# paganpasta/eqxvision

Hardware: AMD Instinct MI355X
Metric: images/sec (higher is better)
Workload: dtype bf16; 1 GPU; resnet50 bf16 forward, batch=256/GPU, 3x224x224, 1000 classes; global_batch=256, parallelism=dp1, graph=True, lanes=2, collective_forced_1rank=False

## Files before the change

eqxvision_amd/build.py:

```python
from __future__ import annotations

import glob
import os
import subprocess
import sys
from concurrent.futures import ThreadPoolExecutor

HERE = os.path.dirname(os.path.abspath(__file__))
CSRC = os.path.join(HERE, "csrc")
LIB = os.path.join(CSRC, "libeqxvision_amd.so")
HIPCC = os.environ.get("HIPCC", "/opt/rocm/bin/hipcc")
FLAGS = ["--offload-arch=gfx950", "-O3", "-std=c++17", "-fPIC", "-Wno-unused-value"]
PROF = bool(os.environ.get("EQV_PROF"))
if PROF:
    FLAGS.append("-DMV_I8_PROF")
    LIB = os.path.join(CSRC, "libeqxvision_amd_prof.so")


def _newer(src, dst):
    return (not os.path.exists(dst)) or os.path.getmtime(src) > os.path.getmtime(dst)


def build(force: bool = False, verbose: bool = True) -> str:
    srcs = sorted(glob.glob(os.path.join(CSRC, "*.hip")))
    hdrs = glob.glob(os.path.join(CSRC, "*.h")) + glob.glob(os.path.join(HERE, "..", "include", "*.h"))
    objdir = os.path.join(CSRC, "build_prof" if PROF else "build")
    os.makedirs(objdir, exist_ok=True)
    newest_hdr = max(os.path.getmtime(h) for h in hdrs)
    jobs = []
    for s in srcs:
        o = os.path.join(objdir, os.path.basename(s)[:-4] + ".o")
        if force or _newer(s, o) or newest_hdr > os.path.getmtime(o):
            jobs.append((s, o))

    def cc(job):
        s, o = job
        cmd = [HIPCC] + FLAGS + ["-c", s, "-o", o]
        r = subprocess.run(cmd, capture_output=True, text=True)
        if r.returncode != 0:
            raise RuntimeError(f"hipcc failed on {s}:\n{r.stderr[-4000:]}")
        return s

    if jobs:
        if verbose:
            print(f"[eqxvision_amd.build] compiling {len(jobs)} file(s) for gfx950", file=sys.stderr)
        with ThreadPoolExecutor(max_workers=min(8, len(jobs))) as ex:
            list(ex.map(cc, jobs))
    objs = [os.path.join(objdir, os.path.basename(s)[:-4] + ".o") for s in srcs]
    if jobs or not os.path.exists(LIB):
        r = subprocess.run([HIPCC, "--offload-arch=gfx950", "-shared", "-fPIC"] + objs + ["-ldl", "-o", LIB],
                           capture_output=True, text=True)
        if r.returncode != 0:
            raise RuntimeError(f"link failed:\n{r.stderr[-4000:]}")
    return LIB


if __name__ == "__main__":
    print(build(force="--force" in sys.argv))
```

eqxvision_amd/csrc/igemm8.hip:

```cpp
#include <type_traits>

#include "igemm_pipe.h"

namespace mv {

namespace {

constexpr unsigned OOB = 0x80000000u;

__device__ unsigned g_dev_status = 0;
constexpr int LDS_W = 0, LDS_XT = 65536, LDS_XB = 98304;
constexpr int LDS_TOTAL = 131072;
constexpr int LDS_LNP = LDS_TOTAL, LN_MAXP = 3, LDS_LNS = LDS_LNP + LN_MAXP * 2048, LDS_TOTAL_LN = LDS_LNS + 2048;
constexpr int LDS_LN_SLOTS = 8 * 32 * (64 * 4 + 16), LDS_LN_DUMMY = LDS_LN_SLOTS + 256 * 32;
static_assert(LDS_LN_DUMMY + 8 * 512 <= LDS_TOTAL, "producer statistics slots");

template <int LOFF>
__device__ __forceinline__ void dma16(unsigned ldsw, unsigned voff, const u32x4& rsrc, unsigned soff) {
    asm volatile("s_add_u32 m0, %0, %4\n\tbuffer_load_dwordx4 %1, %2, %3 offen lds"
                 :
                 : "s"(ldsw), "v"(voff), "s"(rsrc), "s"(soff), "n"(LOFF)
                 : "memory", "scc");
}

template <int LOFF>
__device__ __forceinline__ void dma4(unsigned ldsw, unsigned voff, const u32x4& rsrc, unsigned soff) {
    asm volatile("s_add_u32 m0, %0, %4\n\tbuffer_load_dword %1, %2, %3 offen lds"
                 :
                 : "s"(ldsw), "v"(voff), "s"(rsrc), "s"(soff), "n"(LOFF)
                 : "memory", "scc");
}

__device__ __forceinline__ u32x4 make_rsrc(const void* base) {
    const unsigned long long b = (unsigned long long)base;
    u32x4 r;
    r[0] = __builtin_amdgcn_readfirstlane((unsigned)b);
    r[1] = __builtin_amdgcn_readfirstlane((unsigned)(b >> 32) & 0xffffu);
    r[2] = OOB;
    r[3] = 0x00020000u;
    return r;
}

template <int N> __device__ __forceinline__ void wait_vm_lgkm0() {
    asm volatile("s_waitcnt vmcnt(%0) lgkmcnt(0)" ::"n"(N) : "memory");
}

}

struct TapState {
    int r, s, c0;
    unsigned xoff;
    unsigned woff;
    unsigned bit;
};

__device__ __forceinline__ TapState tap_first() {
    TapState s;
    s.r = 0; s.s = 0; s.c0 = 0; s.xoff = 0; s.woff = 0; s.bit = 1u;
    return s;
}

template <bool DUAL> __device__ __forceinline__ void tap_next(const Igemm2P& p, TapState& s, int tile, int nk1) {
    s.woff += 128u;
    if (DUAL && tile >= nk1) {
        s.xoff = 128u * (unsigned)(tile - nk1);
        return;
    }
    s.c0 += 64;
    if (s.c0 == p.C) {
        s.c0 = 0;
        if (++s.s == p.S) { s.s = 0; ++s.r; }
        s.bit <<= 1;
    }
    s.xoff = 2u * (unsigned)(((s.r * p.dh) * p.W + s.s * p.dw) * p.C + s.c0);
}

template <bool DUAL> __device__ __forceinline__ TapState tap_at(const Igemm2P& p, int tile, int nk1) {
// ... 131 lines not shown
    for (int j = 0; j < 4; ++j) {
        const int n = n0 + 64 * j + 8 * wave + srow;
        wvo[j] = n < p.K ? (unsigned)n * wrow_bytes + 16u * (unsigned)gch : OOB;
    }
    const unsigned lds0 = (unsigned)(uintptr_t)(__attribute__((address_space(3))) char*)smem;
    const unsigned ldsw = __builtin_amdgcn_readfirstlane(lds0 + wave * (8 * ROWB));

    auto tap_adv = [&](TapState& s, int tile) {
        if constexpr (DENSE) { s.woff += 128u; s.xoff += 128u; }
        else tap_next<DUAL>(p, s, tile, nk1);
    };
    auto x_piece = [&](int q, const TapState& s, int tile, auto loff) {
        constexpr int LOFF = decltype(loff)::value;
        if (DUAL && tile >= nk1) {
            if constexpr (DUAL) dma16<LOFF>(ldsw, xvo2[q], rx2, s.xoff);
        } else if constexpr (DENSE) {
            dma16<LOFF>(ldsw, xvo[q], rx, s.xoff);
        } else {
            const unsigned vo = (xmask[q] & s.bit) ? xvo[q] : OOB;
            dma16<LOFF>(ldsw, vo, rx, s.xoff);
        }
    };
#define MV_I8_W(BUF, st)                                                           \
    do {                                                                           \
        dma16<LDS_W + (BUF) * 32768 + 0 * 8192>(ldsw, wvo[0], rw, (st).woff);      \
        dma16<LDS_W + (BUF) * 32768 + 1 * 8192>(ldsw, wvo[1], rw, (st).woff);      \
        dma16<LDS_W + (BUF) * 32768 + 2 * 8192>(ldsw, wvo[2], rw, (st).woff);      \
        dma16<LDS_W + (BUF) * 32768 + 3 * 8192>(ldsw, wvo[3], rw, (st).woff);      \
    } while (0)
#define MV_I8_X(BUF, q, st, tile)                                                                                     \
    x_piece(q, st, tile,                                                                                               \
            std::integral_constant<int, ((q) < 2 ? LDS_XT : LDS_XB) + (BUF) * 16384 + ((q) & 1) * 8192>{})

    const int fr = lane & 31, fh = lane >> 5, swz = (fr >> 1) & 7;
    unsigned waddr[4], xaddr[4];
#pragma unroll
    for (int kk = 0; kk < 4; ++kk) {
        const unsigned ko = (unsigned)(((2 * kk + fh) ^ swz) << 4);
        waddr[kk] = lds0 + LDS_W + (64 * wc + fr) * ROWB + ko;
        xaddr[kk] = lds0 + LDS_XT + (64 * grp + fr) * ROWB + ko;
    }

#ifdef MV_I8_PROF
    const OutT* res = (p.dbg & 8) ? nullptr : (const OutT*)p.residual;
    const bool do_store = !(p.dbg & 4);
#else
    const OutT* res = (const OutT*)p.residual;
    constexpr bool do_store = true;
#endif
    ScaleShift8 ss;
    if constexpr (LIN) ss.load_shift(p.shift, n0 + 64 * wc + (lane & 7) * 8, p.K);
    else ss.load(p.scale, p.shift, n0 + 64 * wc + (lane & 7) * 8, p.K);

    f32x16 acc[2][4];
#pragma unroll
    for (int a = 0; a < 2; ++a)
#pragma unroll
        for (int b = 0; b < 4; ++b)
#pragma unroll
            for (int e = 0; e < 16; ++e) acc[a][b][e] = 0.f;

    TapState sa = tap_first();
    TapState sb = tap_first();
    if constexpr (LNF == 2) {
        const u32x4 rs = make_rsrc(p.stats_in);
        const unsigned ldsw4 = __builtin_amdgcn_readfirstlane(lds0 + wave * 256);
        const unsigned svo = m0 + (tid >> 1) < p.M ? 4u * (unsigned)(2 * m0 + tid) : OOB;
        const unsigned pstep = 8u * (unsigned)p.M;
        const int P = (p.C + 255) >> 8;
#define MV_I8_LNP(j) if ((j) < P) dma4<LDS_LNP + (j) * 2048>(ldsw4, svo, rs, (unsigned)(j) * pstep)
        MV_I8_LNP(0); MV_I8_LNP(1); MV_I8_LNP(2);
#undef MV_I8_LNP
    }
    MV_I8_W(0, sa);
    MV_I8_X(0, 0, sa, 0);
    MV_I8_X(0, 1, sb, 0);
    MV_I8_X(0, 2, sb, 0);
    MV_I8_X(0, 3, sb, 0);
    auto ln_finalize = [&]() {
        __builtin_amdgcn_s_barrier();
        if (tid < 256) {
            const int P = (p.C + 255) >> 8;
            const unsigned a0 = lds0 + LDS_LNP + 8u * (unsigned)tid;
            u32x2 pc[LN_MAXP];
#define MV_I8_RD(j) asm volatile("ds_read_b64 %0, %1 offset:%2" : "=v"(pc[j]) : "v"(a0), "n"((j) * 2048) : "memory")
            MV_I8_RD(0); MV_I8_RD(1); MV_I8_RD(2);
#undef MV_I8_RD
            asm volatile("s_waitcnt lgkmcnt(0)" ::: "memory");
#pragma unroll
            for (int j = 0; j < LN_MAXP; ++j) asm volatile("" : "+v"(pc[j]));
            float tot = 0.f;
#pragma unroll
            for (int j = 0; j < LN_MAXP; ++j) tot += j < P ? __uint_as_float(pc[j][0]) : 0.f;
            const float inv_n = 1.0f / (float)p.C, mean = tot * inv_n;
            float m2 = 0.f;
#pragma unroll
            for (int j = 0; j < LN_MAXP; ++j) {
                const float nj = (float)min(256, p.C - 256 * j);
                const float d = __uint_as_float(pc[j][0]) / nj - mean;
                m2 += j < P ? __uint_as_float(pc[j][1]) + nj * d * d : 0.f;
            }
            const float rstd = 1.0f / sqrtf(m2 * inv_n + p.ln_eps);
            *(float2*)(smem + LDS_LNS + 8 * tid) = make_float2(-mean * rstd, rstd);
        }
    };
    if (nk > 1) {
        tap_adv(sa, 1);
        MV_I8_W(1, sa);
        MV_I8_X(1, 0, sa, 1);
        if constexpr (LNF == 2) { wait_vm<13>(); ln_finalize(); }
        wait_vm<7>();
    } else {
        if constexpr (LNF == 2) { wait_vm<8>(); ln_finalize(); }
        wait_vm<2>();
    }
    __builtin_amdgcn_s_barrier();
    if (grp == 1) __builtin_amdgcn_s_barrier();
#ifdef MV_I8_PROF
    if (p.prof) pt1 = wall_clock64();
#endif
    MV_I8_STAMP();

    u32x4 wf[2][4], xf[2][4];
    auto mfma_half = [&](int half) {
        __builtin_amdgcn_sched_barrier(0);
        __builtin_amdgcn_s_setprio(1);
#pragma unroll
        for (int kk = 0; kk < 4; ++kk)
#pragma unroll
            for (int a = 0; a < 2; ++a)
#pragma unroll
                for (int b = 0; b < 2; ++b)
                    acc[a][2 * half + b] = __builtin_amdgcn_mfma_f32_32x32x16_bf16(
                        __builtin_bit_cast(bf16x8, wf[a][kk]), __builtin_bit_cast(bf16x8, xf[b][kk]), acc[a][2 * half + b], 0, 0, 0);
        __builtin_amdgcn_s_setprio(0);
        __builtin_amdgcn_sched_barrier(0);
    };
    auto pin_frags = [&]() {
#pragma unroll
        for (int kk = 0; kk < 4; ++kk)
            asm volatile("" : "+v"(wf[0][kk]), "+v"(wf[1][kk]), "+v"(xf[0][kk]), "+v"(xf[1][kk]));
    };

    auto ktile = [&](int it, auto bufc) {
        constexpr int BUF = decltype(bufc)::value;
#ifdef MV_I8_PROF
        const bool do_reads = !(p.dbg & 2), do_dma = !(p.dbg & 1);
#else
        constexpr bool do_reads = true, do_dma = true;
#endif
        if (do_reads) {
#pragma unroll
            for (int kk = 0; kk < 4; ++kk) {
                lds_read16<BUF * 32768>(wf[0][kk], waddr[kk]);
                lds_read16<BUF * 32768 + 32 * ROWB>(wf[1][kk], waddr[kk]);
            }
#pragma unroll
            for (int kk = 0; kk < 4; ++kk) {
                lds_read16<BUF * 16384>(xf[0][kk], xaddr[kk]);
                lds_read16<BUF * 16384 + 32 * ROWB>(xf[1][kk], xaddr[kk]);
            }
        }
        if (!do_dma) {
            wait_vm_lgkm0<0>();
        } else if (it + 1 < nk) {
            tap_adv(sb, it + 1);
            MV_I8_X(BUF ^ 1, 1, sb, it + 1);
            MV_I8_X(BUF ^ 1, 2, sb, it + 1);
            MV_I8_X(BUF ^ 1, 3, sb, it + 1);
            wait_vm_lgkm0<8>();
        } else {
            wait_vm_lgkm0<0>();
        }
        pin_frags();
        __builtin_amdgcn_s_barrier();
        MV_I8_STAMP();
        mfma_half(0);
        __builtin_amdgcn_s_barrier();
        MV_I8_STAMP();
        if (do_reads) {
#pragma unroll
            for (int kk = 0; kk < 4; ++kk) {
                lds_read16<(LDS_XB - LDS_XT) + BUF * 16384>(xf[0][kk], xaddr[kk]);
                lds_read16<(LDS_XB - LDS_XT) + BUF * 16384 + 32 * ROWB>(xf[1][kk], xaddr[kk]);
            }
        }
        if (!do_dma) {
            wait_vm_lgkm0<0>();
        } else if (it + 2 < nk) {
            tap_adv(sa, it + 2);
            MV_I8_W(BUF, sa);
            MV_I8_X(BUF, 0, sa, it + 2);
            wait_vm_lgkm0<7>();
        } else if (it + 1 < nk) {
            wait_vm_lgkm0<2>();
        } else {
            wait_vm_lgkm0<0>();
        }
        pin_frags();
        __builtin_amdgcn_s_barrier();
        MV_I8_STAMP();
        mfma_half(1);
        __builtin_amdgcn_s_barrier();
        MV_I8_STAMP();
    };
    for (int it = 0; it < nk; it += 2) {
        ktile(it, std::integral_constant<int, 0>{});
        if (it + 1 < nk) ktile(it + 1, std::integral_constant<int, 1>{});
    }
    if (grp == 0) __builtin_amdgcn_s_barrier();
#ifdef MV_I8_PROF
    if (p.prof) pt2 = wall_clock64();
#endif

    if constexpr (LNF == 0 || LNF == 2)
        epilogue_rows<OutT, LIN, 4, EPITCH, LNF>(p, smem + wave * (32 * EPITCH), acc, ss, res, do_store, m0 + 128 * grp, n0 + 64 * wc, lane,
                                                 smem + LDS_LNS + 1024 * grp);
    else
    {
        epilogue_rows_ln<LNF != 1, LNF != 4, 4, EPITCH>(p, smem + wave * (32 * EPITCH), acc, ss, do_store, m0 + 128 * grp, n0 + 64 * wc, lane,
                                                        smem + LDS_LN_SLOTS + 128 * 32 * grp, wc, smem + LDS_LN_DUMMY + 512 * wave);
        if constexpr (LNF != 4) {
            __syncthreads();
            if (tid < 256 && do_store) merge_row_stats(p, smem + LDS_LN_SLOTS, tid, m0, tile_n, min(4, (p.K - n0) >> 6));
        }
    }
#ifdef MV_I8_PROF
    if (p.prof) {
        if (tid == 0) {
            long long* o = p.prof + 4ll * blockIdx.x;
            o[0] = pt0; o[1] = pt1; o[2] = pt2; o[3] = wall_clock64();
        }
        if (blockIdx.x == 0 && lane == 0) {
            long long* o = p.prof + 4ll * gridDim.x + wave * 128;
            for (int i = 0; i < 128; ++i) o[i] = i < nstamp ? (long long)stamps[i] : -1;
        }
    }
#endif
#undef MV_I8_STAMP
#undef MV_I8_W
#undef MV_I8_X
}

template <typename OutT, int ARR, bool DUAL, bool DENSE = false>
__global__ __launch_bounds__(512) void igemm8s_kernel(const Igemm2P p) {
    static_assert(!(DUAL && DENSE), "DENSE is single-source");
    constexpr int BM = ARR == 0 ? 128 : 256, BN = ARR == 0 ? 256 : 128;
    constexpr int ROWB = 128;
    constexpr int XI = BM / 64, WI = BN / 64;
    constexpr int XBYTES = BM * ROWB;
    constexpr int SLOT = (BM + BN) * ROWB;
    constexpr int EPITCH = 64 * 4 + 16;
    static_assert(XI + WI == 6 && 3 * SLOT <= 160 * 1024 && 8 * 32 * EPITCH <= 3 * SLOT, "ring layout");
// ... 52 lines not shown
        const bool second = DUAL && tile >= nk1;
        if (second) {
            if constexpr (DUAL) {
                dma16<BASE + 0 * 8192>(ldsw, xvo2[0], rx2, st.xoff);
                dma16<BASE + 1 * 8192>(ldsw, xvo2[1], rx2, st.xoff);
                if constexpr (XI == 4) {
                    dma16<BASE + 2 * 8192>(ldsw, xvo2[2], rx2, st.xoff);
                    dma16<BASE + 3 * 8192>(ldsw, xvo2[3], rx2, st.xoff);
                }
            }
        } else if constexpr (DENSE) {
            dma16<BASE + 0 * 8192>(ldsw, xvo[0], rx, st.xoff);
            dma16<BASE + 1 * 8192>(ldsw, xvo[1], rx, st.xoff);
            if constexpr (XI == 4) {
                dma16<BASE + 2 * 8192>(ldsw, xvo[2], rx, st.xoff);
                dma16<BASE + 3 * 8192>(ldsw, xvo[3], rx, st.xoff);
            }
        } else {
            dma16<BASE + 0 * 8192>(ldsw, (xmask[0] & st.bit) ? xvo[0] : OOB, rx, st.xoff);
            dma16<BASE + 1 * 8192>(ldsw, (xmask[1] & st.bit) ? xvo[1] : OOB, rx, st.xoff);
            if constexpr (XI == 4) {
                dma16<BASE + 2 * 8192>(ldsw, (xmask[2] & st.bit) ? xvo[2] : OOB, rx, st.xoff);
                dma16<BASE + 3 * 8192>(ldsw, (xmask[3] & st.bit) ? xvo[3] : OOB, rx, st.xoff);
            }
        }
        dma16<BASE + XBYTES + 0 * 8192>(ldsw, wvo[0], rw, st.woff);
        dma16<BASE + XBYTES + 1 * 8192>(ldsw, wvo[1], rw, st.woff);
        if constexpr (WI == 4) {
            dma16<BASE + XBYTES + 2 * 8192>(ldsw, wvo[2], rw, st.woff);
            dma16<BASE + XBYTES + 3 * 8192>(ldsw, wvo[3], rw, st.woff);
        }
    };

    const int fr = lane & 31, fh = lane >> 5, swz = (fr >> 1) & 7;
    unsigned waddr[4], xaddr[4], waddr2[4], xaddr2[4];
#pragma unroll
    for (int kk = 0; kk < 4; ++kk) {
        const unsigned ko = (unsigned)(((2 * kk + fh) ^ swz) << 4);
        xaddr[kk] = lds0 + (xrow0 + fr) * ROWB + ko;
        waddr[kk] = lds0 + XBYTES + (wrow0 + fr) * ROWB + ko;
        xaddr2[kk] = xaddr[kk] + 2 * SLOT;
        waddr2[kk] = waddr[kk] + 2 * SLOT;
    }

    const OutT* res = (const OutT*)p.residual;
    ScaleShift8 ss;
    ss.load(p.scale, p.shift, n0 + wrow0 + (lane & 7) * 8, p.K);

    f32x16 acc[2][2];
#pragma unroll
    for (int a = 0; a < 2; ++a)
#pragma unroll
        for (int b = 0; b < 2; ++b)
#pragma unroll
            for (int e = 0; e < 16; ++e) acc[a][b][e] = 0.f;

    TapState st = tap_first();
    if (k0) {
        if constexpr (DENSE) { st.woff = st.xoff = 128u * (unsigned)k0; }
        else st = tap_at<DUAL>(p, k0, nk1);
    }
    stage(st, k0, std::integral_constant<int, 0>{});
    if (nk > 1) {
        tap_adv(st, k0 + 1);
        stage(st, k0 + 1, std::integral_constant<int, 1>{});
        wait_vm<6>();
    } else {
        wait_vm<0>();
    }
    __builtin_amdgcn_s_barrier();
    if (grp == 1) __builtin_amdgcn_s_barrier();

    u32x4 wf[2][4], xf[2][4];
    auto ktile = [&](int it, auto slotc) {
        constexpr int SL = decltype(slotc)::value;
        constexpr int OFF = SL == 2 ? 0 : SL * SLOT;
#pragma unroll
        for (int kk = 0; kk < 4; ++kk) {
            lds_read16<OFF>(wf[0][kk], SL == 2 ? waddr2[kk] : waddr[kk]);
            lds_read16<OFF + 32 * ROWB>(wf[1][kk], SL == 2 ? waddr2[kk] : waddr[kk]);
            lds_read16<OFF>(xf[0][kk], SL == 2 ? xaddr2[kk] : xaddr[kk]);
            lds_read16<OFF + 32 * ROWB>(xf[1][kk], SL == 2 ? xaddr2[kk] : xaddr[kk]);
        }
        if (it + 2 < nk) {
            tap_adv(st, k0 + it + 2);
            stage(st, k0 + it + 2, std::integral_constant<int, (SL + 2) % 3>{});
            wait_vm_lgkm0<6>();
        } else {
            wait_vm_lgkm0<0>();
        }
#pragma unroll
        for (int kk = 0; kk < 4; ++kk)
            asm volatile("" : "+v"(wf[0][kk]), "+v"(wf[1][kk]), "+v"(xf[0][kk]), "+v"(xf[1][kk]));
        __builtin_amdgcn_s_barrier();
        __builtin_amdgcn_sched_barrier(0);
        __builtin_amdgcn_s_setprio(1);
#pragma unroll
        for (int kk = 0; kk < 4; ++kk)
#pragma unroll
            for (int a = 0; a < 2; ++a)
#pragma unroll
                for (int b = 0; b < 2; ++b)
                    acc[a][b] = __builtin_amdgcn_mfma_f32_32x32x16_bf16(__builtin_bit_cast(bf16x8, wf[a][kk]),
                                                                        __builtin_bit_cast(bf16x8, xf[b][kk]), acc[a][b], 0, 0, 0);
        __builtin_amdgcn_s_setprio(0);
        __builtin_amdgcn_sched_barrier(0);
        __builtin_amdgcn_s_barrier();
    };
    for (int it = 0; it < nk; it += 3) {
        ktile(it, std::integral_constant<int, 0>{});
        if (it + 1 < nk) ktile(it + 1, std::integral_constant<int, 1>{});
        if (it + 2 < nk) ktile(it + 2, std::integral_constant<int, 2>{});
    }
    if (grp == 0) __builtin_amdgcn_s_barrier();

    if (splitk) {
        unsigned* sync = p.sync + 2 * t;
        float4* part = (float4*)p.ws + (size_t)t * (BM * BN / 4) + tid;
        const unsigned xcc = __builtin_amdgcn_s_getreg(20 | (3 << 11)) & 15u;
        if (tid == 0) *(volatile unsigned*)smem = __hip_atomic_fetch_add(sync, 1u, __ATOMIC_RELAXED, __HIP_MEMORY_SCOPE_AGENT);
        __syncthreads();
        const unsigned arrived = *(volatile unsigned*)smem;
        __syncthreads();
        if (arrived == 0) {
#pragma unroll
            for (int a = 0; a < 2; ++a)
#pragma unroll
                for (int b = 0; b < 2; ++b)
#pragma unroll
                    for (int g = 0; g < 4; ++g)
                        part[((a * 2 + b) * 4 + g) * 512] = make_float4(acc[a][b][4 * g + 0], acc[a][b][4 * g + 1],
                                                                        acc[a][b][4 * g + 2], acc[a][b][4 * g + 3]);
            __syncthreads();
            if (tid == 0) __hip_atomic_store(sync + 1, 1u + xcc, __ATOMIC_RELEASE, __HIP_MEMORY_SCOPE_AGENT);
            return;
        }
        if (tid == 0) {
            int spins = 0;
            unsigned f;
            while ((f = __hip_atomic_load(sync + 1, __ATOMIC_RELAXED, __HIP_MEMORY_SCOPE_AGENT)) == 0u && ++spins < (1 << 20))
                __builtin_amdgcn_s_sleep(2);
            if (f == 0u)
                __hip_atomic_fetch_or(&g_dev_status, 1u, __ATOMIC_RELAXED, __HIP_MEMORY_SCOPE_AGENT);
            if (f != 1u + xcc) __builtin_amdgcn_fence(__ATOMIC_ACQUIRE, "agent");
            __hip_atomic_store(sync, 0u, __ATOMIC_RELAXED, __HIP_MEMORY_SCOPE_AGENT);
            __hip_atomic_store(sync + 1, 0u, __ATOMIC_RELAXED, __HIP_MEMORY_SCOPE_AGENT);
        }
        __syncthreads();
#pragma unroll
        for (int a = 0; a < 2; ++a)
#pragma unroll
            for (int b = 0; b < 2; ++b)
#pragma unroll
                for (int g = 0; g < 4; ++g) {
                    const float4 o = part[((a * 2 + b) * 4 + g) * 512];
                    acc[a][b][4 * g + 0] += o.x; acc[a][b][4 * g + 1] += o.y; acc[a][b][4 * g + 2] += o.z; acc[a][b][4 * g + 3] += o.w;
                }
    }

    epilogue_rows<OutT, false, 2, EPITCH>(p, smem + wave * (32 * EPITCH), acc, ss, res, true, m0 + xrow0, n0 + wrow0, lane);
}

int device_status(int clear, unsigned* out) {
    unsigned v = 0;
    MV_HIP(hipMemcpyFromSymbol(&v, HIP_SYMBOL(g_dev_status), sizeof(v), 0, hipMemcpyDeviceToHost));
    if (clear && v) {
        const unsigned z = 0;
        MV_HIP(hipMemcpyToSymbol(HIP_SYMBOL(g_dev_status), &z, sizeof(z), 0, hipMemcpyHostToDevice));
    }
    *out = v;
    return MV_OK;
}

unsigned* device_status_word() {
    void* p = nullptr;
    if (hipGetSymbolAddress(&p, HIP_SYMBOL(g_dev_status)) != hipSuccess) {
        (void)hipGetLastError();
        return nullptr;
    }
    return (unsigned*)p;
}

size_t splitk_scratch_bytes(long long M, long long N, long long kred) {
    if (N <= 0 || M <= 0) return 0;
    const long long ta = ((M + 127) / 128) * ((N + 255) / 256), tb = ((M + 255) / 256) * ((N + 127) / 128);
    if (!splitk_rule(ta < tb ? ta : tb, kred / 64, get_flag)) return 0;
    return SPLITK_SYNC_BYTES + (size_t)(ta > tb ? ta : tb) * 128 * 256 * 4;
}

static int igemm8_go(Igemm2P& p, bool dual, bool out_f32, int tile, hipStream_t st) {
    const int bm = tile == 1 ? 128 : 256, bn = tile == 2 ? 128 : 256;
    p.tiles_m = (p.M + bm - 1) / bm;
    p.tiles_n = (p.K + bn - 1) / bn;
// ... 157 lines not shown
```

eqxvision_amd/csrc/igemm_pipe.h:

```cpp
#pragma once
#include "mfma_common.h"

namespace mv {

struct Igemm2P {
    const bf16_t* x;
    const bf16_t* w;
    const float* scale;
    const float* shift;
    const void* residual;
    void* y;
    const bf16_t* zero;
    int N, H, W, C, K, R, S, Ho, Wo, sh, sw, ph, pw, dh, dw;
    int M, tiles_m, tiles_n, act;
    int dbg;
    long long* prof;
    const bf16_t* x2;
    int C2, H2, W2, s2;
    int gm;
    int skew;
    int tok;
    unsigned* sync;
    float* ws;
    void* y2;
    const void* residual2;
    float* stats_out;
    const float* stats_in;
    float ln_eps;
};

typedef unsigned int u32x4 __attribute__((ext_vector_type(4)));
typedef unsigned int u32x2 __attribute__((ext_vector_type(2)));

template <int IMM> __device__ __forceinline__ void lds_read16(u32x4& dst, unsigned addr) {
    asm volatile("ds_read_b128 %0, %1 offset:%2" : "=v"(dst) : "v"(addr), "n"(IMM) : "memory");
}
template <int N> __device__ __forceinline__ void wait_vm() { asm volatile("s_waitcnt vmcnt(%0)" ::"n"(N) : "memory"); }

template <typename OutT> struct R8;
template <> struct R8<bf16_t> {
    uint4 u;
    __device__ __forceinline__ void load(const bf16_t* p) { u = *(const uint4*)p; }
    __device__ __forceinline__ void add_to(float* v) const {
        const uint32_t w[4] = {u.x, u.y, u.z, u.w};
#pragma unroll
        for (int e = 0; e < 4; ++e) {
            v[2 * e] += __uint_as_float(w[e] << 16);
            v[2 * e + 1] += __uint_as_float(w[e] & 0xffff0000u);
        }
    }
};
template <> struct R8<float> {
    float4 a, b;
    __device__ __forceinline__ void load(const float* p) { a = *(const float4*)p; b = *(const float4*)(p + 4); }
    __device__ __forceinline__ void add_to(float* v) const {
        v[0] += a.x; v[1] += a.y; v[2] += a.z; v[3] += a.w; v[4] += b.x; v[5] += b.y; v[6] += b.z; v[7] += b.w;
    }
};


template <typename OutT> struct Buf8;
template <> struct Buf8<bf16_t> {
    u32x4 u;
    __device__ __forceinline__ void load(brsrc_t r, unsigned vo, unsigned so) { u = __builtin_amdgcn_raw_buffer_load_b128(r, vo, so, 0); }
    __device__ __forceinline__ void add_to(float* v) const {
// ... 8 lines not shown
        o[0] = pack_bf2(v[0], v[1]); o[1] = pack_bf2(v[2], v[3]); o[2] = pack_bf2(v[4], v[5]); o[3] = pack_bf2(v[6], v[7]);
        __builtin_amdgcn_raw_buffer_store_b128(o, r, vo, 0, 0);
    }
};
template <> struct Buf8<float> {
    u32x4 a, b;
    __device__ __forceinline__ void load(brsrc_t r, unsigned vo, unsigned so) {
        a = __builtin_amdgcn_raw_buffer_load_b128(r, vo, so, 0);
        b = __builtin_amdgcn_raw_buffer_load_b128(r, vo + 16u, so, 0);
    }
    __device__ __forceinline__ void add_to(float* v) const {
#pragma unroll
        for (int e = 0; e < 4; ++e) { v[e] += __uint_as_float(a[e]); v[4 + e] += __uint_as_float(b[e]); }
    }
    static __device__ __forceinline__ void store(brsrc_t r, unsigned vo, const float* v) {
        u32x4 lo, hi;
#pragma unroll
        for (int e = 0; e < 4; ++e) { lo[e] = __float_as_uint(v[e]); hi[e] = __float_as_uint(v[4 + e]); }
        __builtin_amdgcn_raw_buffer_store_b128(lo, r, vo, 0, 0);
        __builtin_amdgcn_raw_buffer_store_b128(hi, r, vo + 16u, 0, 0);
    }
};

__device__ __forceinline__ float dpp_xor1(float v) { return __builtin_bit_cast(float, __builtin_amdgcn_update_dpp(0, __builtin_bit_cast(int, v), 0xB1, 0xf, 0xf, true)); }
__device__ __forceinline__ float dpp_xor2(float v) { return __builtin_bit_cast(float, __builtin_amdgcn_update_dpp(0, __builtin_bit_cast(int, v), 0x4E, 0xf, 0xf, true)); }
__device__ __forceinline__ float dpp_half_mirror(float v) { return __builtin_bit_cast(float, __builtin_amdgcn_update_dpp(0, __builtin_bit_cast(int, v), 0x141, 0xf, 0xf, true)); }
__device__ __forceinline__ float sum8_lanes(float v) {
    v += dpp_xor1(v);
    v += dpp_xor2(v);
    v += dpp_half_mirror(v);
    return v;
}

template <typename OutT, bool LIN, int NBT, int EPITCH, int LNF = 0>
__device__ __forceinline__ void epilogue_rows(const Igemm2P& p, char* ep, f32x16 (&acc)[2][NBT], const ScaleShift8& ss,
                                              const OutT* res, bool do_store, int mrow0, int ncol0, int lane,
                                              const char* lnst = nullptr) {
    static_assert(LNF == 0 || (LNF == 2 && sizeof(OutT) == 2 && !LIN), "LayerNorm fold, consumer form");
    constexpr unsigned SZ = sizeof(OutT);
    const int fr = lane & 31, fh = lane >> 5, r0 = lane >> 3, c8 = lane & 7;
    const int rl = ncol0 + c8 * 8 < p.K ? p.M - mrow0 : 0;
    const long long wave_elem = (long long)mrow0 * p.K + ncol0;
    const bool has_res = res != nullptr;
    const brsrc_t rr = make_brsrc(has_res ? res + wave_elem : (const OutT*)p.y, has_res);
    const unsigned vrow = (unsigned)(r0 * p.K + c8 * 8) * SZ;
    const unsigned kstep = 8u * (unsigned)p.K * SZ;
    const bool hm = p.tok > 0;
    int bi0 = 0, ti0 = 0;
    if (hm) { bi0 = mrow0 / p.tok; ti0 = mrow0 - bi0 * p.tok; }
    const long long y_elem = hm ? ((long long)bi0 * (p.K >> 6) + (ncol0 >> 6)) * p.tok * 64 : wave_elem;
    const brsrc_t ry = make_brsrc((OutT*)p.y + y_elem, do_store);
    const float inv_tok = hm ? 1.0f / (float)p.tok : 0.f;
    const unsigned img_step = (unsigned)(p.K >> 6) * (unsigned)p.tok * 64u;
    auto row_vo = [&](int row) -> unsigned { return row + r0 < rl ? vrow : BUF_OOB; };
    auto y_vo = [&](int row, int step) -> unsigned {
        unsigned rel = vrow + (unsigned)step * kstep;
        if (hm) {
            const int v = ti0 + row + r0;
            int q = (int)((float)v * inv_tok), t = v - q * p.tok;
            q += t >= p.tok ? 1 : (t < 0 ? -1 : 0);
            t -= t >= p.tok ? p.tok : (t < 0 ? -p.tok : 0);
            rel = ((unsigned)q * img_step + (unsigned)t * 64u + (unsigned)c8 * 8u) * SZ;
        }
        return row + r0 < rl ? rel : BUF_OOB;
    };
    Buf8<OutT> late[2][4];
    auto fetch_res = [&](int b, Buf8<OutT>(&dst)[4]) {
#pragma unroll
        for (int pass = 0; pass < 4; ++pass) dst[pass].load(rr, row_vo(b * 32 + pass * 8), (unsigned)(b * 4 + pass) * kstep);
    };
    fetch_res(0, late[0]);
#pragma unroll
    for (int b = 0; b < NBT; ++b) {
        if (b + 1 < NBT) fetch_res(b + 1, late[(b + 1) & 1]);
#pragma unroll
        for (int a = 0; a < 2; ++a)
#pragma unroll
            for (int g = 0; g < 4; ++g) {
                const int nl = a * 32 + 8 * g + 4 * fh;
                *(float4*)(ep + fr * EPITCH + nl * 4) = make_float4(acc[a][b][4 * g + 0], acc[a][b][4 * g + 1],
                                                                     acc[a][b][4 * g + 2], acc[a][b][4 * g + 3]);
            }
        wave_lds_fence();
#pragma unroll
        for (int pass = 0; pass < 4; ++pass) {
            const int row = pass * 8 + r0;
            const float4 lo = *(const float4*)(ep + row * EPITCH + c8 * 32);
            const float4 hi = *(const float4*)(ep + row * EPITCH + c8 * 32 + 16);
            float v[8] = {lo.x, lo.y, lo.z, lo.w, hi.x, hi.y, hi.z, hi.w};
            if constexpr (LNF == 2) {
                const float2 st = *(const float2*)(lnst + (b * 32 + row) * 8);
#pragma unroll
                for (int e = 0; e < 8; ++e) v[e] = fmaf(st.y, v[e], fmaf(st.x, ss.sc[e], ss.sh[e]));
            } else if constexpr (LIN) ss.apply_shift(v);
            else ss.apply(v);
            if (has_res) late[b & 1][pass].add_to(v);
            const unsigned voy = y_vo(b * 32 + pass * 8, b * 4 + pass);
            if (p.act == MV_ACT_RELU) {
#pragma unroll
                for (int e = 0; e < 8; ++e) v[e] = fmaxf(v[e], 0.f);
            }
            if constexpr (sizeof(OutT) == 2) {
                u32x4 o;
                if (p.act == MV_ACT_GELU_TANH) {
                    o[0] = gelu_tanh_pack2(v[0], v[1]); o[1] = gelu_tanh_pack2(v[2], v[3]);
                    o[2] = gelu_tanh_pack2(v[4], v[5]); o[3] = gelu_tanh_pack2(v[6], v[7]);
                } else {
                    o[0] = pack_bf2(v[0], v[1]); o[1] = pack_bf2(v[2], v[3]); o[2] = pack_bf2(v[4], v[5]); o[3] = pack_bf2(v[6], v[7]);
                }
                __builtin_amdgcn_raw_buffer_store_b128(o, ry, voy, 0, 0);
            } else {
                if (p.act == MV_ACT_GELU_TANH) {
#pragma unroll
                    for (int e = 0; e < 8; ++e) v[e] = gelu_tanh_f(v[e]);
                }
                Buf8<OutT>::store(ry, voy, v);
            }
        }
        wave_lds_fence();
    }
}


template <bool RES_SPLIT, bool OUT_SPLIT, int NBT, int EPITCH>
__device__ __forceinline__ void epilogue_rows_ln(const Igemm2P& p, char* ep, f32x16 (&acc)[2][NBT], const ScaleShift8& ss, bool do_store,
                                                 int mrow0, int ncol0, int lane, char* slots, int wc, char* dummy) {
    static_assert(RES_SPLIT || OUT_SPLIT, "fp32 in, fp32 out is the plain epilogue");
    const int fr = lane & 31, fh = lane >> 5, r0 = lane >> 3, c8 = lane & 7;
    const int rl = ncol0 + c8 * 8 < p.K ? p.M - mrow0 : 0;
    const long long wave_elem = (long long)mrow0 * p.K + ncol0;
    const unsigned vrow2 = (unsigned)(r0 * p.K + c8 * 8) * 2u, kstep2 = 16u * (unsigned)p.K;
    const brsrc_t rra = make_brsrc(RES_SPLIT ? (const void*)((const bf16_t*)p.residual + wave_elem) : (const void*)((const float*)p.residual + wave_elem));
    const brsrc_t rrb = make_brsrc(RES_SPLIT ? (const void*)((const bf16_t*)p.residual2 + wave_elem) : (const void*)p.y, RES_SPLIT);
    const brsrc_t rya = make_brsrc(OUT_SPLIT ? (void*)((bf16_t*)p.y + wave_elem) : (void*)((float*)p.y + wave_elem), do_store);
    const brsrc_t ryb = make_brsrc(OUT_SPLIT ? (void*)((bf16_t*)p.y2 + wave_elem) : p.y, OUT_SPLIT && do_store);
    auto row_ok = [&](int row) -> bool { return row + r0 < rl; };
    u32x4 la[2][4], lb[2][4];
    auto fetch_res = [&](int b, u32x4 (&da)[4], u32x4 (&db)[4]) {
#pragma unroll
        for (int pass = 0; pass < 4; ++pass) {
            const bool ok = row_ok(b * 32 + pass * 8);
            const unsigned step = (unsigned)(b * 4 + pass);
            if constexpr (RES_SPLIT) {
                da[pass] = __builtin_amdgcn_raw_buffer_load_b128(rra, ok ? vrow2 : BUF_OOB, step * kstep2, 0);
                db[pass] = __builtin_amdgcn_raw_buffer_load_b128(rrb, ok ? vrow2 : BUF_OOB, step * kstep2, 0);
            } else {
                da[pass] = __builtin_amdgcn_raw_buffer_load_b128(rra, ok ? 2u * vrow2 : BUF_OOB, step * 2u * kstep2, 0);
                db[pass] = __builtin_amdgcn_raw_buffer_load_b128(rra, ok ? 2u * vrow2 + 16u : BUF_OOB, step * 2u * kstep2, 0);
            }
        }
    };
    fetch_res(0, la[0], lb[0]);
#pragma unroll
    for (int b = 0; b < NBT; ++b) {
        if (b + 1 < NBT) fetch_res(b + 1, la[(b + 1) & 1], lb[(b + 1) & 1]);
#pragma unroll
        for (int a = 0; a < 2; ++a)
#pragma unroll
            for (int g = 0; g < 4; ++g) {
                const int nl = a * 32 + 8 * g + 4 * fh;
                *(float4*)(ep + fr * EPITCH + nl * 4) = make_float4(acc[a][b][4 * g + 0], acc[a][b][4 * g + 1],
                                                                     acc[a][b][4 * g + 2], acc[a][b][4 * g + 3]);
            }
        wave_lds_fence();
#pragma unroll
        for (int pass = 0; pass < 4; ++pass) {
            const int row = pass * 8 + r0;
            const float4 lo = *(const float4*)(ep + row * EPITCH + c8 * 32);
            const float4 hi = *(const float4*)(ep + row * EPITCH + c8 * 32 + 16);
            float v[8] = {lo.x, lo.y, lo.z, lo.w, hi.x, hi.y, hi.z, hi.w};
            ss.apply_shift(v);
            const u32x4 ra = la[b & 1][pass], rb = lb[b & 1][pass];
#pragma unroll
            for (int e = 0; e < 4; ++e) {
                if constexpr (RES_SPLIT) {
                    v[2 * e] += __uint_as_float(ra[e] << 16) + __uint_as_float(rb[e] << 16);
                    v[2 * e + 1] += __uint_as_float(ra[e] & 0xffff0000u) + __uint_as_float(rb[e] & 0xffff0000u);
                } else {
                    v[e] += __uint_as_float(ra[e]);
                    v[4 + e] += __uint_as_float(rb[e]);
                }
            }
            const bool ok = row_ok(b * 32 + pass * 8);
            const unsigned step = (unsigned)(b * 4 + pass);
            if constexpr (OUT_SPLIT) {
                const float s = sum8_lanes(((v[0] + v[1]) + (v[2] + v[3])) + ((v[4] + v[5]) + (v[6] + v[7])));
                const float mu = s * (1.0f / 64.0f);
                float q = 0.f;
#pragma unroll
                for (int e = 0; e < 8; ++e) { const float d = v[e] - mu; q = fmaf(d, d, q); }
                q = sum8_lanes(q);
                *(float2*)(c8 == 0 ? slots + ((b * 32 + row) * 4 + wc) * 8 : dummy + lane * 8) = make_float2(s, q);
                u32x4 oh, ol;
#pragma unroll
                for (int e = 0; e < 4; ++e) {
                    oh[e] = pack_bf2(v[2 * e], v[2 * e + 1]);
// ... 35 lines not shown
```

Before: 90620 images/s.

## Switch implicit-GEMM inner loop from 32x32x16 to 16x16x32 bf16 MFMA

```diff
diff --git a/eqxvision_amd/build.py b/eqxvision_amd/build.py
--- a/eqxvision_amd/build.py
+++ b/eqxvision_amd/build.py
@@ -15,6 +15,11 @@
 if PROF:
     FLAGS.append("-DMV_I8_PROF")
     LIB = os.path.join(CSRC, "libeqxvision_amd_prof.so")
+OBJDIR = "build_prof" if PROF else "build"
+if os.environ.get("EQV_I8_M16") == "0":
+    FLAGS.append("-DMV_I8_M16=0")
+    LIB = LIB[:-3] + "_m32.so"
+    OBJDIR += "_m32"
 
 
 def _newer(src, dst):
@@ -24,7 +29,7 @@
 def build(force: bool = False, verbose: bool = True) -> str:
     srcs = sorted(glob.glob(os.path.join(CSRC, "*.hip")))
     hdrs = glob.glob(os.path.join(CSRC, "*.h")) + glob.glob(os.path.join(HERE, "..", "include", "*.h"))
-    objdir = os.path.join(CSRC, "build_prof" if PROF else "build")
+    objdir = os.path.join(CSRC, OBJDIR)
     os.makedirs(objdir, exist_ok=True)
     newest_hdr = max(os.path.getmtime(h) for h in hdrs)
     jobs = []
diff --git a/eqxvision_amd/csrc/igemm8.hip b/eqxvision_amd/csrc/igemm8.hip
--- a/eqxvision_amd/csrc/igemm8.hip
+++ b/eqxvision_amd/csrc/igemm8.hip
@@ -1,6 +1,10 @@
 #include <type_traits>
 
 #include "igemm_pipe.h"
+
+#ifndef MV_I8_M16
+#define MV_I8_M16 1
+#endif
 
 namespace mv {
 
@@ -43,6 +47,17 @@
 
 template <int N> __device__ __forceinline__ void wait_vm_lgkm0() {
     asm volatile("s_waitcnt vmcnt(%0) lgkmcnt(0)" ::"n"(N) : "memory");
+}
+
+constexpr bool M16 = MV_I8_M16 != 0;
+constexpr int FROWS = M16 ? 16 : 32, FT = 64 / FROWS, KS = M16 ? 2 : 4, FCH = 8 / KS, LAY = M16 ? 1 : 0;
+using acc_t = std::conditional_t<M16, f32x4, f32x16>;
+__device__ __forceinline__ acc_t mfma_step(const u32x4& w, const u32x4& x, const acc_t& c) {
+#if MV_I8_M16
+    return __builtin_amdgcn_mfma_f32_16x16x32_bf16(__builtin_bit_cast(bf16x8, w), __builtin_bit_cast(bf16x8, x), c, 0, 0, 0);
+#else
+    return __builtin_amdgcn_mfma_f32_32x32x16_bf16(__builtin_bit_cast(bf16x8, w), __builtin_bit_cast(bf16x8, x), c, 0, 0, 0);
+#endif
 }
 
 }
@@ -240,11 +255,11 @@
     x_piece(q, st, tile,                                                                                               \
             std::integral_constant<int, ((q) < 2 ? LDS_XT : LDS_XB) + (BUF) * 16384 + ((q) & 1) * 8192>{})
 
-    const int fr = lane & 31, fh = lane >> 5, swz = (fr >> 1) & 7;
-    unsigned waddr[4], xaddr[4];
-#pragma unroll
-    for (int kk = 0; kk < 4; ++kk) {
-        const unsigned ko = (unsigned)(((2 * kk + fh) ^ swz) << 4);
+    const int fr = lane & (FROWS - 1), fh = lane / FROWS, swz = (fr >> 1) & 7;
+    unsigned waddr[KS], xaddr[KS];
+#pragma unroll
+    for (int kk = 0; kk < KS; ++kk) {
+        const unsigned ko = (unsigned)(((FCH * kk + fh) ^ swz) << 4);
         waddr[kk] = lds0 + LDS_W + (64 * wc + fr) * ROWB + ko;
         xaddr[kk] = lds0 + LDS_XT + (64 * grp + fr) * ROWB + ko;
     }
@@ -260,13 +275,13 @@
     if constexpr (LIN) ss.load_shift(p.shift, n0 + 64 * wc + (lane & 7) * 8, p.K);
     else ss.load(p.scale, p.shift, n0 + 64 * wc + (lane & 7) * 8, p.K);
 
-    f32x16 acc[2][4];
-#pragma unroll
-    for (int a = 0; a < 2; ++a)
-#pragma unroll
-        for (int b = 0; b < 4; ++b)
-#pragma unroll
-            for (int e = 0; e < 16; ++e) acc[a][b][e] = 0.f;
+    acc_t acc[FT][2 * FT];
+#pragma unroll
+    for (int a = 0; a < FT; ++a)
+#pragma unroll
+        for (int b = 0; b < 2 * FT; ++b)
+#pragma unroll
+            for (int e = 0; e < (int)(sizeof(acc_t) / 4); ++e) acc[a][b][e] = 0.f;
 
     TapState sa = tap_first();
     TapState sb = tap_first();
@@ -329,25 +344,38 @@
 #endif
     MV_I8_STAMP();
 
-    u32x4 wf[2][4], xf[2][4];
+    u32x4 wf[FT][KS], xf[FT][KS];
     auto mfma_half = [&](int half) {
         __builtin_amdgcn_sched_barrier(0);
         __builtin_amdgcn_s_setprio(1);
 #pragma unroll
-        for (int kk = 0; kk < 4; ++kk)
-#pragma unroll
-            for (int a = 0; a < 2; ++a)
-#pragma unroll
-                for (int b = 0; b < 2; ++b)
-                    acc[a][2 * half + b] = __builtin_amdgcn_mfma_f32_32x32x16_bf16(
-                        __builtin_bit_cast(bf16x8, wf[a][kk]), __builtin_bit_cast(bf16x8, xf[b][kk]), acc[a][2 * half + b], 0, 0, 0);
+        for (int kk = 0; kk < KS; ++kk)
+#pragma unroll
+            for (int a = 0; a < FT; ++a)
+#pragma unroll
+                for (int b = 0; b < FT; ++b)
+                    acc[a][FT * half + b] = mfma_step(wf[a][kk], xf[b][kk], acc[a][FT * half + b]);
         __builtin_amdgcn_s_setprio(0);
         __builtin_amdgcn_sched_barrier(0);
     };
     auto pin_frags = [&]() {
 #pragma unroll
-        for (int kk = 0; kk < 4; ++kk)
-            asm volatile("" : "+v"(wf[0][kk]), "+v"(wf[1][kk]), "+v"(xf[0][kk]), "+v"(xf[1][kk]));
+        for (int kk = 0; kk < KS; ++kk)
+#pragma unroll
+            for (int t = 0; t < FT; t += 2)
+                asm volatile("" : "+v"(wf[t][kk]), "+v"(wf[t + 1][kk]), "+v"(xf[t][kk]), "+v"(xf[t + 1][kk]));
+    };
+    auto read_frags = [&](u32x4 (&f)[FT][KS], const unsigned (&addr)[KS], auto basec) {
+        constexpr int BASE = decltype(basec)::value;
+#pragma unroll
+        for (int kk = 0; kk < KS; ++kk) {
+            lds_read16<BASE>(f[0][kk], addr[kk]);
+            lds_read16<BASE + FROWS * ROWB>(f[1][kk], addr[kk]);
+            if constexpr (FT == 4) {
+                lds_read16<BASE + 2 * FROWS * ROWB>(f[2][kk], addr[kk]);
+                lds_read16<BASE + 3 * FROWS * ROWB>(f[3][kk], addr[kk]);
+            }
+        }
     };
 
     auto ktile = [&](int it, auto bufc) {
@@ -358,16 +386,8 @@
         constexpr bool do_reads = true, do_dma = true;
 #endif
         if (do_reads) {
-#pragma unroll
-            for (int kk = 0; kk < 4; ++kk) {
-                lds_read16<BUF * 32768>(wf[0][kk], waddr[kk]);
-                lds_read16<BUF * 32768 + 32 * ROWB>(wf[1][kk], waddr[kk]);
-            }
-#pragma unroll
-            for (int kk = 0; kk < 4; ++kk) {
-                lds_read16<BUF * 16384>(xf[0][kk], xaddr[kk]);
-                lds_read16<BUF * 16384 + 32 * ROWB>(xf[1][kk], xaddr[kk]);
-            }
+            read_frags(wf, waddr, std::integral_constant<int, BUF * 32768>{});
+            read_frags(xf, xaddr, std::integral_constant<int, BUF * 16384>{});
         }
         if (!do_dma) {
             wait_vm_lgkm0<0>();
@@ -386,13 +406,7 @@
         mfma_half(0);
         __builtin_amdgcn_s_barrier();
         MV_I8_STAMP();
-        if (do_reads) {
-#pragma unroll
-            for (int kk = 0; kk < 4; ++kk) {
-                lds_read16<(LDS_XB - LDS_XT) + BUF * 16384>(xf[0][kk], xaddr[kk]);
-                lds_read16<(LDS_XB - LDS_XT) + BUF * 16384 + 32 * ROWB>(xf[1][kk], xaddr[kk]);
-            }
-        }
+        if (do_reads) read_frags(xf, xaddr, std::integral_constant<int, (LDS_XB - LDS_XT) + BUF * 16384>{});
         if (!do_dma) {
             wait_vm_lgkm0<0>();
         } else if (it + 2 < nk) {
@@ -422,11 +436,11 @@
 #endif
 
     if constexpr (LNF == 0 || LNF == 2)
-        epilogue_rows<OutT, LIN, 4, EPITCH, LNF>(p, smem + wave * (32 * EPITCH), acc, ss, res, do_store, m0 + 128 * grp, n0 + 64 * wc, lane,
+        epilogue_rows<OutT, LIN, 4, EPITCH, LNF, LAY>(p, smem + wave * (32 * EPITCH), acc, ss, res, do_store, m0 + 128 * grp, n0 + 64 * wc, lane,
                                                  smem + LDS_LNS + 1024 * grp);
     else
     {
-        epilogue_rows_ln<LNF != 1, LNF != 4, 4, EPITCH>(p, smem + wave * (32 * EPITCH), acc, ss, do_store, m0 + 128 * grp, n0 + 64 * wc, lane,
+        epilogue_rows_ln<LNF != 1, LNF != 4, 4, EPITCH, LAY>(p, smem + wave * (32 * EPITCH), acc, ss, do_store, m0 + 128 * grp, n0 + 64 * wc, lane,
                                                         smem + LDS_LN_SLOTS + 128 * 32 * grp, wc, smem + LDS_LN_DUMMY + 512 * wave);
         if constexpr (LNF != 4) {
             __syncthreads();
@@ -545,11 +559,11 @@
         }
     };
 
-    const int fr = lane & 31, fh = lane >> 5, swz = (fr >> 1) & 7;
-    unsigned waddr[4], xaddr[4], waddr2[4], xaddr2[4];
-#pragma unroll
-    for (int kk = 0; kk < 4; ++kk) {
-        const unsigned ko = (unsigned)(((2 * kk + fh) ^ swz) << 4);
+    const int fr = lane & (FROWS - 1), fh = lane / FROWS, swz = (fr >> 1) & 7;
+    unsigned waddr[KS], xaddr[KS], waddr2[KS], xaddr2[KS];
+#pragma unroll
+    for (int kk = 0; kk < KS; ++kk) {
+        const unsigned ko = (unsigned)(((FCH * kk + fh) ^ swz) << 4);
         xaddr[kk] = lds0 + (xrow0 + fr) * ROWB + ko;
         waddr[kk] = lds0 + XBYTES + (wrow0 + fr) * ROWB + ko;
         xaddr2[kk] = xaddr[kk] + 2 * SLOT;
@@ -560,13 +574,13 @@
     ScaleShift8 ss;
     ss.load(p.scale, p.shift, n0 + wrow0 + (lane & 7) * 8, p.K);
 
-    f32x16 acc[2][2];
-#pragma unroll
-    for (int a = 0; a < 2; ++a)
-#pragma unroll
-        for (int b = 0; b < 2; ++b)
-#pragma unroll
-            for (int e = 0; e < 16; ++e) acc[a][b][e] = 0.f;
+    acc_t acc[FT][FT];
+#pragma unroll
+    for (int a = 0; a < FT; ++a)
+#pragma unroll
+        for (int b = 0; b < FT; ++b)
+#pragma unroll
+            for (int e = 0; e < (int)(sizeof(acc_t) / 4); ++e) acc[a][b][e] = 0.f;
 
     TapState st = tap_first();
     if (k0) {
@@ -584,16 +598,25 @@
     __builtin_amdgcn_s_barrier();
     if (grp == 1) __builtin_amdgcn_s_barrier();
 
-    u32x4 wf[2][4], xf[2][4];
+    u32x4 wf[FT][KS], xf[FT][KS];
     auto ktile = [&](int it, auto slotc) {
         constexpr int SL = decltype(slotc)::value;
         constexpr int OFF = SL == 2 ? 0 : SL * SLOT;
 #pragma unroll
-        for (int kk = 0; kk < 4; ++kk) {
-            lds_read16<OFF>(wf[0][kk], SL == 2 ? waddr2[kk] : waddr[kk]);
-            lds_read16<OFF + 32 * ROWB>(wf[1][kk], SL == 2 ? waddr2[kk] : waddr[kk]);
-            lds_read16<OFF>(xf[0][kk], SL == 2 ? xaddr2[kk] : xaddr[kk]);
-            lds_read16<OFF + 32 * ROWB>(xf[1][kk], SL == 2 ? xaddr2[kk] : xaddr[kk]);
+        for (int kk = 0; kk < KS; ++kk) {
+            const unsigned wa = SL == 2 ? waddr2[kk] : waddr[kk], xa = SL == 2 ? xaddr2[kk] : xaddr[kk];
+            lds_read16<OFF>(wf[0][kk], wa);
+            lds_read16<OFF + FROWS * ROWB>(wf[1][kk], wa);
+            if constexpr (FT == 4) {
+                lds_read16<OFF + 2 * FROWS * ROWB>(wf[2][kk], wa);
+                lds_read16<OFF + 3 * FROWS * ROWB>(wf[3][kk], wa);
+            }
+            lds_read16<OFF>(xf[0][kk], xa);
+            lds_read16<OFF + FROWS * ROWB>(xf[1][kk], xa);
+            if constexpr (FT == 4) {
+                lds_read16<OFF + 2 * FROWS * ROWB>(xf[2][kk], xa);
+                lds_read16<OFF + 3 * FROWS * ROWB>(xf[3][kk], xa);
+            }
         }
         if (it + 2 < nk) {
             tap_adv(st, k0 + it + 2);
@@ -603,19 +626,19 @@
             wait_vm_lgkm0<0>();
         }
 #pragma unroll
-        for (int kk = 0; kk < 4; ++kk)
-            asm volatile("" : "+v"(wf[0][kk]), "+v"(wf[1][kk]), "+v"(xf[0][kk]), "+v"(xf[1][kk]));
+        for (int kk = 0; kk < KS; ++kk)
+#pragma unroll
+            for (int t = 0; t < FT; t += 2)
+                asm volatile("" : "+v"(wf[t][kk]), "+v"(wf[t + 1][kk]), "+v"(xf[t][kk]), "+v"(xf[t + 1][kk]));
         __builtin_amdgcn_s_barrier();
         __builtin_amdgcn_sched_barrier(0);
         __builtin_amdgcn_s_setprio(1);
 #pragma unroll
-        for (int kk = 0; kk < 4; ++kk)
-#pragma unroll
-            for (int a = 0; a < 2; ++a)
-#pragma unroll
-                for (int b = 0; b < 2; ++b)
-                    acc[a][b] = __builtin_amdgcn_mfma_f32_32x32x16_bf16(__builtin_bit_cast(bf16x8, wf[a][kk]),
-                                                                        __builtin_bit_cast(bf16x8, xf[b][kk]), acc[a][b], 0, 0, 0);
+        for (int kk = 0; kk < KS; ++kk)
+#pragma unroll
+            for (int a = 0; a < FT; ++a)
+#pragma unroll
+                for (int b = 0; b < FT; ++b) acc[a][b] = mfma_step(wf[a][kk], xf[b][kk], acc[a][b]);
         __builtin_amdgcn_s_setprio(0);
         __builtin_amdgcn_sched_barrier(0);
         __builtin_amdgcn_s_barrier();
@@ -636,14 +659,15 @@
         const unsigned arrived = *(volatile unsigned*)smem;
         __syncthreads();
         if (arrived == 0) {
-#pragma unroll
-            for (int a = 0; a < 2; ++a)
-#pragma unroll
-                for (int b = 0; b < 2; ++b)
-#pragma unroll
-                    for (int g = 0; g < 4; ++g)
-                        part[((a * 2 + b) * 4 + g) * 512] = make_float4(acc[a][b][4 * g + 0], acc[a][b][4 * g + 1],
-                                                                        acc[a][b][4 * g + 2], acc[a][b][4 * g + 3]);
+            constexpr int QT = sizeof(acc_t) / 16;
+#pragma unroll
+            for (int a = 0; a < FT; ++a)
+#pragma unroll
+                for (int b = 0; b < FT; ++b)
+#pragma unroll
+                    for (int g = 0; g < QT; ++g)
+                        part[((a * FT + b) * QT + g) * 512] = make_float4(acc[a][b][4 * g + 0], acc[a][b][4 * g + 1],
+                                                                          acc[a][b][4 * g + 2], acc[a][b][4 * g + 3]);
             __syncthreads();
             if (tid == 0) __hip_atomic_store(sync + 1, 1u + xcc, __ATOMIC_RELEASE, __HIP_MEMORY_SCOPE_AGENT);
             return;
@@ -660,18 +684,19 @@
             __hip_atomic_store(sync + 1, 0u, __ATOMIC_RELAXED, __HIP_MEMORY_SCOPE_AGENT);
         }
         __syncthreads();
-#pragma unroll
-        for (int a = 0; a < 2; ++a)
-#pragma unroll
-            for (int b = 0; b < 2; ++b)
-#pragma unroll
-                for (int g = 0; g < 4; ++g) {
-                    const float4 o = part[((a * 2 + b) * 4 + g) * 512];
+        constexpr int QT = sizeof(acc_t) / 16;
+#pragma unroll
+        for (int a = 0; a < FT; ++a)
+#pragma unroll
+            for (int b = 0; b < FT; ++b)
+#pragma unroll
+                for (int g = 0; g < QT; ++g) {
+                    const float4 o = part[((a * FT + b) * QT + g) * 512];
                     acc[a][b][4 * g + 0] += o.x; acc[a][b][4 * g + 1] += o.y; acc[a][b][4 * g + 2] += o.z; acc[a][b][4 * g + 3] += o.w;
                 }
     }
 
-    epilogue_rows<OutT, false, 2, EPITCH>(p, smem + wave * (32 * EPITCH), acc, ss, res, true, m0 + xrow0, n0 + wrow0, lane);
+    epilogue_rows<OutT, false, 2, EPITCH, 0, LAY>(p, smem + wave * (32 * EPITCH), acc, ss, res, true, m0 + xrow0, n0 + wrow0, lane);
 }
 
 int device_status(int clear, unsigned* out) {
diff --git a/eqxvision_amd/csrc/igemm_pipe.h b/eqxvision_amd/csrc/igemm_pipe.h
--- a/eqxvision_amd/csrc/igemm_pipe.h
+++ b/eqxvision_amd/csrc/igemm_pipe.h
@@ -31,6 +31,7 @@
 
 typedef unsigned int u32x4 __attribute__((ext_vector_type(4)));
 typedef unsigned int u32x2 __attribute__((ext_vector_type(2)));
+typedef float f32x4 __attribute__((ext_vector_type(4)));
 
 template <int IMM> __device__ __forceinline__ void lds_read16(u32x4& dst, unsigned addr) {
     asm volatile("ds_read_b128 %0, %1 offset:%2" : "=v"(dst) : "v"(addr), "n"(IMM) : "memory");
@@ -105,13 +106,28 @@
     return v;
 }
 
-template <typename OutT, bool LIN, int NBT, int EPITCH, int LNF = 0>
-__device__ __forceinline__ void epilogue_rows(const Igemm2P& p, char* ep, f32x16 (&acc)[2][NBT], const ScaleShift8& ss,
+template <int EPITCH, typename AccT>
+__device__ __forceinline__ void patch_write16(char* ep, const AccT& acc, int b, int lane) {
+    const int fr = lane & 15, fq = lane >> 4;
+#pragma unroll
+    for (int t = 0; t < 2; ++t)
+#pragma unroll
+        for (int a = 0; a < 4; ++a) {
+            const int nl = a * 16 + 4 * fq;
+            *(float4*)(ep + (16 * t + fr) * EPITCH + nl * 4) = make_float4(acc[a][2 * b + t][0], acc[a][2 * b + t][1],
+                                                                            acc[a][2 * b + t][2], acc[a][2 * b + t][3]);
+        }
+}
+
+template <typename OutT, bool LIN, int NBT, int EPITCH, int LNF = 0, int LAY = 0, typename AccT>
+__device__ __forceinline__ void epilogue_rows(const Igemm2P& p, char* ep, AccT& acc, const ScaleShift8& ss,
                                               const OutT* res, bool do_store, int mrow0, int ncol0, int lane,
                                               const char* lnst = nullptr) {
     static_assert(LNF == 0 || (LNF == 2 && sizeof(OutT) == 2 && !LIN), "LayerNorm fold, consumer form");
+    static_assert(sizeof(AccT) == NBT * 32 * sizeof(float), "NBT x 32 registers per lane");
     constexpr unsigned SZ = sizeof(OutT);
     const int fr = lane & 31, fh = lane >> 5, r0 = lane >> 3, c8 = lane & 7;
+    (void)fr; (void)fh;
     const int rl = ncol0 + c8 * 8 < p.K ? p.M - mrow0 : 0;
     const long long wave_elem = (long long)mrow0 * p.K + ncol0;
     const bool has_res = res != nullptr;
@@ -146,14 +162,19 @@
 #pragma unroll
     for (int b = 0; b < NBT; ++b) {
         if (b + 1 < NBT) fetch_res(b + 1, late[(b + 1) & 1]);
-#pragma unroll
-        for (int a = 0; a < 2; ++a)
-#pragma unroll
-            for (int g = 0; g < 4; ++g) {
-                const int nl = a * 32 + 8 * g + 4 * fh;
-                *(float4*)(ep + fr * EPITCH + nl * 4) = make_float4(acc[a][b][4 * g + 0], acc[a][b][4 * g + 1],
-                                                                     acc[a][b][4 * g + 2], acc[a][b][4 * g + 3]);
-            }
+        if constexpr (LAY == 0) {
+#pragma unroll
+            for (int a = 0; a < 2; ++a)
+#pragma unroll
+                for (int g = 0; g < 4; ++g) {
+                    const int nl = a * 32 + 8 * g + 4 * fh;
+                    *(float4*)(ep + fr * EPITCH + nl * 4) = make_float4(acc[a][b][4 * g + 0], acc[a][b][4 * g + 1],
+                                                                         acc[a][b][4 * g + 2], acc[a][b][4 * g + 3]);
+                }
+        } else {
+            static_assert(LAY == 1, "accumulator layout");
+            patch_write16<EPITCH>(ep, acc, b, lane);
+        }
         wave_lds_fence();
 #pragma unroll
         for (int pass = 0; pass < 4; ++pass) {
@@ -195,11 +216,13 @@
 }
 
 
-template <bool RES_SPLIT, bool OUT_SPLIT, int NBT, int EPITCH>
-__device__ __forceinline__ void epilogue_rows_ln(const Igemm2P& p, char* ep, f32x16 (&acc)[2][NBT], const ScaleShift8& ss, bool do_store,
+template <bool RES_SPLIT, bool OUT_SPLIT, int NBT, int EPITCH, int LAY = 0, typename AccT>
+__device__ __forceinline__ void epilogue_rows_ln(const Igemm2P& p, char* ep, AccT& acc, const ScaleShift8& ss, bool do_store,
                                                  int mrow0, int ncol0, int lane, char* slots, int wc, char* dummy) {
     static_assert(RES_SPLIT || OUT_SPLIT, "fp32 in, fp32 out is the plain epilogue");
+    static_assert(sizeof(AccT) == NBT * 32 * sizeof(float), "NBT x 32 registers per lane");
     const int fr = lane & 31, fh = lane >> 5, r0 = lane >> 3, c8 = lane & 7;
+    (void)fr; (void)fh;
     const int rl = ncol0 + c8 * 8 < p.K ? p.M - mrow0 : 0;
     const long long wave_elem = (long long)mrow0 * p.K + ncol0;
     const unsigned vrow2 = (unsigned)(r0 * p.K + c8 * 8) * 2u, kstep2 = 16u * (unsigned)p.K;
@@ -227,14 +250,19 @@
 #pragma unroll
     for (int b = 0; b < NBT; ++b) {
         if (b + 1 < NBT) fetch_res(b + 1, la[(b + 1) & 1], lb[(b + 1) & 1]);
-#pragma unroll
-        for (int a = 0; a < 2; ++a)
-#pragma unroll
-            for (int g = 0; g < 4; ++g) {
-                const int nl = a * 32 + 8 * g + 4 * fh;
-                *(float4*)(ep + fr * EPITCH + nl * 4) = make_float4(acc[a][b][4 * g + 0], acc[a][b][4 * g + 1],
-                                                                     acc[a][b][4 * g + 2], acc[a][b][4 * g + 3]);
-            }
+        if constexpr (LAY == 0) {
+#pragma unroll
+            for (int a = 0; a < 2; ++a)
+#pragma unroll
+                for (int g = 0; g < 4; ++g) {
+                    const int nl = a * 32 + 8 * g + 4 * fh;
+                    *(float4*)(ep + fr * EPITCH + nl * 4) = make_float4(acc[a][b][4 * g + 0], acc[a][b][4 * g + 1],
+                                                                         acc[a][b][4 * g + 2], acc[a][b][4 * g + 3]);
+                }
+        } else {
+            static_assert(LAY == 1, "accumulator layout");
+            patch_write16<EPITCH>(ep, acc, b, lane);
+        }
         wave_lds_fence();
 #pragma unroll
         for (int pass = 0; pass < 4; ++pass) {
```

Result: no change. 90410 images/s (-0.2%).
